# suhrig/arriba

Hardware: AMD Instinct MI355X
Metric: chimeric reads/s end-to-end (BAM->fusions.tsv), synthetic (higher is better)
Workload: dtype int32

## Files before the change

### arriba_amd/csrc/device/agpu_ingest.hip

```cpp
#include <hip/hip_runtime.h>
#include <algorithm>
#include <cstring>
#include <string>
#include <vector>
#include <rocprim/rocprim.hpp>
#include "agpu_context.hpp"
#include "ingest_core.hpp"
#include "device_utils.hpp"
#include "shard_host.hpp"
#include "crc32_core.hpp"
#include "inflate_fast_core.hpp"

using namespace agpu;
namespace agpu { extern thread_local bool g_inside_ingest_finish; }

namespace {

const int BLOCK = 256;
inline unsigned int grid_for(uint64_t n, int block = BLOCK) { return (unsigned int) ((n + block - 1) / block); }

enum { IC_ACTIVE = 0, IC_MAPPED_READS = 1, IC_MISSING_HI = 2, IC_BROKEN = 3, IC_MALFORMED = 4, IC_CHIMERIC = 5, IC_COLLISION = 6, IC_MISMATCH = 7, IC_UNSORTED = 8, IC_MAX_NAME = 9,
       IC_MAX_READ_LENGTH = 10, IC_STRAND_COUNT = 11, IC_STRAND_MATCHING = 12, IC_RUNS_UNSORTED = 13, IC_QNAME_COMMA = 14, IC_COUNT = 16 };

#define HIP_CHECK(call) do { hipError_t e_ = (call); if (e_ != hipSuccess) { set_last_error(std::string(#call) + ": " + hipGetErrorString(e_)); return AGPU_ERR_DEVICE; } } while (0)
// ... 204 lines not shown
__global__ void run_key_kernel(const uint64_t* keys, const uint32_t* group_first, uint32_t n_groups, uint64_t* out) {
	const uint32_t g = blockIdx.x * BLOCK + threadIdx.x;
	if (g < n_groups) out[g] = keys[group_first[g]];
}
__global__ void run_repeat_kernel(const uint64_t* sorted_keys, uint32_t n_groups, uint32_t* repeats) {
	__shared__ uint32_t block_sum;
	uint32_t mine = 0;
	for (uint64_t g = blockIdx.x * (uint64_t) BLOCK + threadIdx.x; g < n_groups; g += gridDim.x * (uint64_t) BLOCK) mine += g > 0 && sorted_keys[g] == sorted_keys[g - 1];
	block_tally(mine, repeats, &block_sum);
}

struct ViralCounter {
	unsigned long long* counts;
	__device__ void operator()(uint32_t contig) { atomicAdd(&counts[contig], 1ull); }
};

#ifndef AGPU_REPLAY_WAVES
#define AGPU_REPLAY_WAVES 0
#endif
#ifndef AGPU_PACK_WAVES
#define AGPU_PACK_WAVES 0
#endif
#if AGPU_REPLAY_WAVES > 0
#define AGPU_REPLAY_OCCUPANCY __attribute__((amdgpu_waves_per_eu(AGPU_REPLAY_WAVES, AGPU_REPLAY_WAVES)))
#else
#define AGPU_REPLAY_OCCUPANCY
#endif
#if AGPU_PACK_WAVES > 0
#define AGPU_PACK_OCCUPANCY __attribute__((amdgpu_waves_per_eu(AGPU_PACK_WAVES, AGPU_PACK_WAVES)))
#else
#define AGPU_PACK_OCCUPANCY
#endif
template <bool RUNS, int ROLE = ROLE_WHOLE> __global__ void __launch_bounds__(BLOCK) AGPU_REPLAY_OCCUPANCY group_replay_kernel(IngestContext ctx, const uint32_t* sorted_records, const uint32_t* group_begin, const uint32_t* group_count, uint32_t first_group, uint32_t n_groups,
                                                             FragmentPlan* plain, TandemPlan* itd, uint8_t* valid, FragmentSizes* sizes, unsigned long long* viral_counts, uint32_t* qname_differs, uint32_t* counters, TakenNames taken) {
	__shared__ uint32_t sums[2];
	GroupTally tally; tally.malformed = 0; tally.chimeric = 0; tally.collision = 0;
	const uint32_t g = first_group + blockIdx.x * BLOCK + threadIdx.x;
	if (g < n_groups) {
		const uint32_t begin = group_begin[g];
		const uint32_t n_records = group_count[g];
		const Rec representative = load_record(ctx.stream, sorted_records[begin]);
		const int64_t hit = hit_index_of(ctx.stream, sorted_records[begin], representative);
		const uint32_t length = qname_length(representative);
		if (RUNS) {
			if (find_byte(representative.name, length, ',') < length) atomicOr(&counters[IC_QNAME_COMMA], 1u);
			if (g == 0) qname_differs[0] = 0;
			else {
				const uint32_t record_before = sorted_records[group_begin[g - 1]];
				const Rec run_before = load_record(ctx.stream, record_before);
				const uint32_t length_before = qname_length(run_before), shorter = length < length_before ? length : length_before, different = first_difference(run_before.name, representative.name, shorter);
				qname_differs[g] = length != length_before || different < shorter;
				bool unsorted;
				if (different < shorter) unsorted = run_before.name[different] > representative.name[different];
				else unsorted = compare_names(fragment_name(run_before, hit_index_of(ctx.stream, record_before, run_before), false, length_before), fragment_name(representative, hit, false, length)) >= 0;
				if (unsorted) atomicOr(&counters[IC_RUNS_UNSORTED], 1u);
			}
		}
		FragmentPlan plain_plan; TandemPlan itd_plan;
		ViralCounter viral = { viral_counts };
		replay_group_as<ROLE>(ctx, sorted_records + begin, n_records, plain_plan, itd_plan, tally, viral, RUNS ? &representative : nullptr, length, hit, taken);
		if (tally.collision) atomicOr(&counters[IC_COLLISION], 1u);
		Fragment3 fragment;
		AGPU_NOUNROLL for (uint32_t entry = 0; entry < 2; ++entry) {
			const FragmentPlan& plan = entry ? itd_plan.plan : plain_plan;
			bool ok = false;
			if (plan.count > 0) {
				ok = normalize_plan(ctx.stream, plan, entry ? &itd_plan.tandem : nullptr, fragment);
				if (!ok) tally.malformed++;
			}
			valid[2 * (size_t) g + entry] = ok;
			FragmentSizes mine; mine.cigar_words = 0; mine.sequence_bytes = 0; mine.name_length = 0;
			if (ok) { if (entry) itd[g] = itd_plan; else plain[g] = plain_plan; fragment_sizes(fragment, representative, hit, entry, mine, length); }
			sizes[2 * (size_t) g + entry] = mine;
		}
	}
	block_tally(tally.malformed, &counters[IC_MALFORMED], &sums[0]);
	block_tally(tally.chimeric, &counters[IC_CHIMERIC], &sums[1]);
}


__device__ FragmentName name_of(const IngestStream& in, const uint32_t* group_first, uint32_t ref, Rec& storage) {
	storage = load_record(in, group_first[ref >> 1]);
	return fragment_name(storage, hit_index_of(in, group_first[ref >> 1], storage), ref & 1);
}

__global__ void name_order_check_kernel(IngestStream in, const uint32_t* group_first, const uint32_t* order, uint64_t n, uint32_t* counters) {
	__shared__ uint32_t block_max;
	if (threadIdx.x == 0) block_max = 0;
	__syncthreads();
	const uint64_t i = blockIdx.x * (uint64_t) BLOCK + threadIdx.x;
	if (i < n) {
		Rec storage_a, storage_b;
		const FragmentName mine = name_of(in, group_first, order[i], storage_a);
		atomicMax(&block_max, name_length(mine));
		if (i > 0) {
			const FragmentName before = name_of(in, group_first, order[i - 1], storage_b);
			if (compare_names(before, mine) >= 0) atomicOr(&counters[IC_UNSORTED], 1u);
		}
	}
	__syncthreads();
	if (threadIdx.x == 0 && block_max) atomicMax(&counters[IC_MAX_NAME], block_max);
}

__global__ void run_itd_order_kernel(IngestStream in, const uint32_t* group_first, const uint8_t* valid, uint32_t first_group, uint32_t n_groups, uint32_t* counters) {
	const uint32_t g = first_group + blockIdx.x * BLOCK + threadIdx.x;
// ... 1 lines not shown
	Rec storage_a, storage_b;
	const FragmentName mine = name_of(in, group_first, 2 * g, storage_b);
	const FragmentName before = name_of(in, group_first, 2 * (g - 1) + 1, storage_a);
	if (compare_names(before, mine) >= 0) atomicOr(&counters[IC_RUNS_UNSORTED], 1u);
}

__global__ void name_chunk_kernel(IngestStream in, const uint32_t* group_first, const uint32_t* order, uint64_t n, uint32_t chunk, uint64_t* keys) {
	const uint64_t i = blockIdx.x * (uint64_t) BLOCK + threadIdx.x;
	if (i >= n) return;
	Rec storage;
	keys[i] = name_chunk(name_of(in, group_first, order[i], storage), chunk);
}


__global__ void fragment_layout_kernel(IngestStream in, const uint32_t* group_first, const uint32_t* order, uint64_t n, const FragmentSizes* sizes, const uint32_t* qname_run ,
                                       uint32_t* cigar_words, uint32_t* sequence_bytes, uint32_t* name_lengths, uint32_t* new_group) {
	const uint64_t i = blockIdx.x * (uint64_t) BLOCK + threadIdx.x;
	if (i > n) return;
	if (i == n) { cigar_words[i] = 0; sequence_bytes[i] = 0; name_lengths[i] = 0; return; }
	const uint32_t ref = order[i];
	const FragmentSizes mine = sizes[ref];
	cigar_words[i] = mine.cigar_words; sequence_bytes[i] = mine.sequence_bytes; name_lengths[i] = mine.name_length;
	uint32_t differs = 0;
	if (i > 0 && qname_run != nullptr) differs = qname_run[ref >> 1] != qname_run[order[i - 1] >> 1];
	else if (i > 0) {
		const Rec a = load_record(in, group_first[ref >> 1]), b = load_record(in, group_first[order[i - 1] >> 1]);
		const uint32_t length = qname_length(a);
		differs = length != qname_length(b);
		for (uint32_t k = 0; k < length && !differs; ++k) differs = a.name[k] != b.name[k];
	}
	new_group[i] = differs;
}

__global__ void __launch_bounds__(BLOCK) AGPU_PACK_OCCUPANCY fragment_pack_kernel(IngestStream in, const uint32_t* group_first, const uint32_t* order, uint64_t n, const FragmentPlan* plain, const TandemPlan* itd,
                                                              const uint64_t* cigar_base, const uint64_t* sequence_base, const uint64_t* name_base, const uint32_t* group_id, PackTarget out, uint32_t* counters) {
	__shared__ uint32_t block_max;
	if (threadIdx.x == 0) block_max = 0;
	__syncthreads();
	const uint64_t i = blockIdx.x * (uint64_t) BLOCK + threadIdx.x;
	if (i == n) out.name_offset[n] = name_base[n];
	if (i < n) {
		const uint32_t ref = order[i], g = ref >> 1;
		const bool is_itd = ref & 1;
		Fragment3 f;
		normalize_plan(in, is_itd ? itd[g].plan : plain[g], is_itd ? &itd[g].tandem : nullptr, f);
		Rec storage;
		const FragmentName name = name_of(in, group_first, ref, storage);
		atomicMax(&block_max, write_fragment(in, f, name, i, cigar_base[i], sequence_base[i], name_base[i], group_id[i], out));
	}
	__syncthreads();
	if (threadIdx.x == 0 && block_max) atomicMax(&counters[IC_MAX_READ_LENGTH], block_max);
}

template <bool INFLATED> __global__ void __launch_bounds__(256) bgzf_crc_kernel(const uint8_t* raw, const agpu_bgzf_block* blocks, uint32_t n_blocks, const Crc32Tables* tables, unsigned int* mismatches) {
	__shared__ uint32_t slice[4][256];
	__shared__ uint32_t join[2][4][256];
	__shared__ uint32_t staged[4][CRC32_WAVE_LANES * (CRC32_ROUND_WORDS + 1)];
	for (uint32_t k = threadIdx.x; k < 4 * 256; k += 256) ((uint32_t*) slice)[k] = ((const uint32_t*) tables->slice)[k];
	for (uint32_t k = threadIdx.x; k < 2 * 4 * 256; k += 256) ((uint32_t*) join)[k] = ((const uint32_t*) tables->join)[k];
	const uint32_t wave = threadIdx.x / CRC32_WAVE_LANES, lane = threadIdx.x % CRC32_WAVE_LANES, b = blockIdx.x * 4 + wave;
	agpu_bgzf_block block;
	block.crc32 = 0; block.payload_size = 0; block.raw_offset = 0; block.payload_offset = 0;
	if (b < n_blocks) block = blocks[b];
	if (INFLATED) { block.raw_offset = block.stream_offset; block.payload_offset = 0; block.payload_size = block.isize; }
	const bool checked = b < n_blocks && block.crc32 != 0 && block.payload_size <= CRC32_VIRTUAL;
	const uint8_t* payload = raw + block.raw_offset + block.payload_offset;
	const uint32_t n = block.payload_size;
	uint32_t* mine = staged[wave];
	uint32_t c = 0;
	const bool by_chunks = checked && n >= 4;
	const uint32_t first_word = by_chunks ? (CRC32_VIRTUAL - n) / 4 : CRC32_VIRTUAL / 4;
	for (uint32_t round = 0; round < CRC32_WAVE_CHUNK / 4 / CRC32_ROUND_WORDS; ++round) {
		__syncthreads();
		for (uint32_t item = lane; item < CRC32_WAVE_LANES * CRC32_ROUND_WORDS; item += CRC32_WAVE_LANES) {
			const uint32_t chunk = item / CRC32_ROUND_WORDS, j = item % CRC32_ROUND_WORDS, w = chunk * (CRC32_WAVE_CHUNK / 4) + round * CRC32_ROUND_WORDS + j;
			mine[chunk * (CRC32_ROUND_WORDS + 1) + j] = w >= first_word ? crc32_virtual_word(payload, n, w) : 0u;
		}
		__syncthreads();
		for (uint32_t j = 0; j < CRC32_ROUND_WORDS; ++j) c = crc32_raw_step(slice, c, mine[lane * (CRC32_ROUND_WORDS + 1) + j]);
	}
	__syncthreads();
// ... 262 lines not shown
		const uint64_t records = w.record_end - w.record_begin;
		w.active_begin = p.active;
		if (records == 0) break;
		DeviceBuffer& record_offset = ctx->scratch("ingest.record_offset"); DeviceBuffer& keys = ctx->scratch("ingest.keys"); DeviceBuffer& record_bits = ctx->scratch("ingest.record_bits"); DeviceBuffer& active_records = ctx->scratch("ingest.sorted_records");
		TRY(grow_keeping(ctx, record_offset, w.record_end * 8, w.record_begin * 8, estimated_records * 8)); TRY(grow_keeping(ctx, keys, w.record_end * 8, w.record_begin * 8, estimated_records * 8));
		TRY(grow_keeping(ctx, ctx->scratch("ingest.hit_index"), w.record_end * 4, w.record_begin * 4, estimated_records * 4));
		TRY(grow_keeping(ctx, record_bits, w.record_end, w.record_begin, estimated_records)); TRY(grow_keeping(ctx, active_records, (w.active_begin + records) * 4, w.active_begin * 4, estimated_records * 4));
		{ KernelTimer timer(ctx, "segment_emit_kernel", records * 8, s);
		  segment_emit_kernel<<<grid_for(n), BLOCK, 0, s>>>(bytes, w.avail, base, w.segment_begin, w.segment_end, ctx->scratch("ingest.segment_first").as<uint64_t>(), ctx->scratch("ingest.segment_base").as<uint32_t>(), record_offset.as<uint64_t>()); }
		const IngestStream in = window_stream(ctx, w.avail, w.record_end);
		{ KernelTimer timer(ctx, "record_parse_kernel", records * (8 + 64 + 9), s);
		  record_parse_kernel<ROLE_WHOLE><<<tally_grid(records, BLOCK) * 8, BLOCK, 0, s>>>(in, ctx->genome, 0, w.record_begin, keys.as<uint64_t>(), record_bits.as<uint8_t>(), ctx->scratch("ingest.hit_index").as<int32_t>(), device_counters); }
		auto flags = rocprim::make_transform_iterator(record_bits.as<uint8_t>() + w.record_begin, RecordIsActive());
		HIP_CHECK(rocprim::select(nullptr, temporary, rocprim::counting_iterator<uint32_t>((uint32_t) w.record_begin), flags, active_records.as<uint32_t>() + w.active_begin, words + 2, records, s));
		if (temporary > rocprim_scratch.capacity) ALLOC(rocprim_scratch, temporary);
		HIP_CHECK(rocprim::select(rocprim_scratch.ptr, temporary, rocprim::counting_iterator<uint32_t>((uint32_t) w.record_begin), flags, active_records.as<uint32_t>() + w.active_begin, words + 2, records, s));
		break; }
	case 3: {
		const uint64_t active = w.active_end - w.active_begin;
		w.head_begin = p.heads;
		if (active == 0) break;
		DeviceBuffer& head = ctx->scratch("ingest.head"); DeviceBuffer& run_begin = ctx->scratch("ingest.group_begin");
		TRY(grow_keeping(ctx, head, w.active_end, 0, estimated_records)); TRY(grow_keeping(ctx, run_begin, (w.head_begin + active + 1) * 4, w.head_begin * 4, estimated_records * 2));
		{ KernelTimer timer(ctx, "run_head_kernel", active * (8 + 4 + 1), s);
		  run_head_kernel<<<grid_for(active), BLOCK, 0, s>>>(ctx->scratch("ingest.keys").as<uint64_t>(), ctx->scratch("ingest.sorted_records").as<uint32_t>(), w.active_begin, w.active_end, head.as<uint8_t>()); }
		HIP_CHECK(rocprim::select(nullptr, temporary, rocprim::counting_iterator<uint32_t>((uint32_t) w.active_begin), head.as<uint8_t>() + w.active_begin, run_begin.as<uint32_t>() + w.head_begin, words + 3, active, s));
		if (temporary > rocprim_scratch.capacity) ALLOC(rocprim_scratch, temporary);
		HIP_CHECK(rocprim::select(rocprim_scratch.ptr, temporary, rocprim::counting_iterator<uint32_t>((uint32_t) w.active_begin), head.as<uint8_t>() + w.active_begin, run_begin.as<uint32_t>() + w.head_begin, words + 3, active, s));
		break; }
	case 4: {
		const uint64_t first_group = p.groups_done, n_groups = w.last ? w.head_end : (w.head_end > 0 ? w.head_end - 1 : 0);
		if (n_groups <= first_group) break;
		DeviceBuffer& group_first = ctx->scratch("ingest.group_first"); DeviceBuffer& group_count = ctx->scratch("ingest.group_count");
		DeviceBuffer& plain = ctx->scratch("ingest.plain_plans"); DeviceBuffer& itd = ctx->scratch("ingest.itd_plans"); DeviceBuffer& valid = ctx->scratch("ingest.valid"); DeviceBuffer& sizes = ctx->scratch("ingest.sizes");
		const size_t estimated_groups = estimated_records / 3;
		TRY(grow_keeping(ctx, group_first, n_groups * 4, first_group * 4, estimated_groups * 4)); TRY(grow_keeping(ctx, group_count, n_groups * 4, first_group * 4, estimated_groups * 4));
		TRY(grow_keeping(ctx, plain, n_groups * sizeof(FragmentPlan), first_group * sizeof(FragmentPlan), estimated_groups * sizeof(FragmentPlan))); TRY(grow_keeping(ctx, itd, n_groups * sizeof(TandemPlan), first_group * sizeof(TandemPlan), estimated_groups * sizeof(TandemPlan)));
		TRY(grow_keeping(ctx, valid, 2 * n_groups, 2 * first_group, 2 * estimated_groups)); TRY(grow_keeping(ctx, sizes, 2 * n_groups * sizeof(FragmentSizes), 2 * first_group * sizeof(FragmentSizes), 2 * estimated_groups * sizeof(FragmentSizes)));
		const uint32_t* active_records = ctx->scratch("ingest.sorted_records").as<uint32_t>(); const uint32_t* run_begin = ctx->scratch("ingest.group_begin").as<uint32_t>();
		const uint64_t groups = n_groups - first_group;
		run_close_kernel<<<grid_for(groups), BLOCK, 0, s>>>(active_records, run_begin, (uint32_t) first_group, (uint32_t) n_groups, (uint32_t) w.head_end, w.active_end, group_first.as<uint32_t>(), group_count.as<uint32_t>());
		const IngestStream in = window_stream(ctx, w.avail, w.record_end);
		DeviceBuffer& qname_differs = ctx->scratch("ingest.qname_differs");
		TRY(grow_keeping(ctx, qname_differs, n_groups * 4, first_group * 4, estimated_groups * 4));
		{ KernelTimer timer(ctx, "group_replay_kernel", n * SEGMENT_BYTES, s);
		  group_replay_kernel<true><<<grid_for(groups), BLOCK, 0, s>>>(replay_context(ctx, in), active_records, run_begin, group_count.as<uint32_t>(), (uint32_t) first_group, (uint32_t) n_groups, plain.as<FragmentPlan>(), itd.as<TandemPlan>(), valid.as<uint8_t>(),
		                                                              sizes.as<FragmentSizes>(), ctx->ingest_viral_counts.as<unsigned long long>(), qname_differs.as<uint32_t>(), device_counters, TakenNames()); }
		{ KernelTimer timer(ctx, "run_itd_order_kernel", groups * 2, s);
		  run_itd_order_kernel<<<grid_for(groups), BLOCK, 0, s>>>(in, group_first.as<uint32_t>(), valid.as<uint8_t>(), (uint32_t) first_group, (uint32_t) n_groups, device_counters); }
		p.groups_done = n_groups; p.touched = true;
		break; }
	}
	HIP_CHECK(hipMemcpyAsync(p.host_words + (size_t) w.slot * INGEST_WINDOW_WORDS, words, INGEST_WINDOW_WORDS * 4, hipMemcpyDeviceToHost, s));
	HIP_CHECK(hipEventRecord(w.readback, s));
	++w.enqueued;
	return AGPU_OK;
}

void window_note(agpu_ctx* ctx, IngestWindow& w) {
	IngestProgress& p = ctx->ingest_progress;
	const uint32_t* words = p.host_words + (size_t) w.slot * INGEST_WINDOW_WORDS;
	w.known = w.enqueued;
	switch (w.known) {
	case 1: {
		w.record_begin = p.records;
		if (w.segment_end == w.segment_begin) { w.record_end = p.records; break; }
		const uint64_t last_end = (uint64_t) words[4] | (uint64_t) words[5] << 32;
		if (words[0] != 0 || last_end >= OFFSET_BROKEN || (w.last && last_end != w.avail)) { p.abandoned = true; break; }
		w.record_end = words[1]; p.records = w.record_end;
		break; }
	case 2: w.active_end = w.active_begin + (w.record_end > w.record_begin ? words[2] : 0); p.active = w.active_end; break;
	case 3: w.head_end = w.head_begin + (w.active_end > w.active_begin ? words[3] : 0); p.heads = w.head_end; break;
	}
}

int windows_advance(agpu_ctx* ctx, bool wait) {
	IngestProgress& p = ctx->ingest_progress;
	while (!p.abandoned && !p.windows.empty()) {
		bool moved = false;
// ... 487 lines not shown
			TRY(sort_pairs<uint64_t>(ctx, rocprim_scratch, keys.as<uint64_t>(), keys_sorted.as<uint64_t>(), nullptr, sorted_records.as<uint32_t>(), n_records, 64, "rocprim::radix_sort_pairs(record keys)", true));
		}
		TRY(read_counters());
		if (host_counters[IC_BROKEN] > 0) { set_last_error(ctx->ingest_role == AGPU_ROLE_SEPARATE_CHIMERIC ? "failed to load alignments: a record of the separate chimeric file (-c) is damaged or has no reference sequence" : "failed to load alignments"); return AGPU_ERR_INVALID; }
		n_active = host_counters[IC_ACTIVE];
		n_groups = 0;
		if (n_active > 0) {
			ALLOC(head, n_active); ALLOC(group_start, (n_active + 1) * 4);
			{ KernelTimer timer(ctx, "group_head_kernel", n_active * (8 + 1));
			  group_head_kernel<<<grid_for(n_active), BLOCK, 0, s>>>(keys_sorted.as<uint64_t>(), n_active, head.as<uint8_t>()); }
			TRY(select_flagged(ctx, rocprim_scratch, head.as<uint8_t>(), group_start.as<uint32_t>(), device_counters + IC_MAX_NAME , n_active));
			TRY(read_counters());
			n_groups = host_counters[IC_MAX_NAME];
			HIP_CHECK(hipMemsetAsync(device_counters + IC_MAX_NAME, 0, 4, s));
			ALLOC(first_flags, n_records); ALLOC(stream_rank, (n_records + 1) * 4); ALLOC(group_first, (size_t) n_groups * 4); ALLOC(group_begin, (size_t) n_groups * 4); ALLOC(group_count, (size_t) n_groups * 4);
			HIP_CHECK(hipMemsetAsync(first_flags.ptr, 0, n_records, s));
			group_first_flag_kernel<<<grid_for(n_groups), BLOCK, 0, s>>>(sorted_records.as<uint32_t>(), group_start.as<uint32_t>(), n_groups, first_flags.as<uint8_t>());
			{ size_t scan_bytes = 0;
			  HIP_CHECK(rocprim::exclusive_scan(nullptr, scan_bytes, first_flags.as<uint8_t>(), stream_rank.as<uint32_t>(), 0u, n_records, rocprim::plus<uint32_t>(), s));
			  if (scan_bytes > rocprim_scratch.capacity) ALLOC(rocprim_scratch, scan_bytes);
			  KernelTimer timer(ctx, "rocprim::exclusive_scan(first records)", n_records * 5);
			  HIP_CHECK(rocprim::exclusive_scan(rocprim_scratch.ptr, scan_bytes, first_flags.as<uint8_t>(), stream_rank.as<uint32_t>(), 0u, n_records, rocprim::plus<uint32_t>(), s)); }
			{ KernelTimer timer(ctx, "group_rank_kernel", (uint64_t) n_groups * 24);
			  group_rank_kernel<<<grid_for(n_groups), BLOCK, 0, s>>>(sorted_records.as<uint32_t>(), group_start.as<uint32_t>(), n_groups, n_active, stream_rank.as<uint32_t>(), group_first.as<uint32_t>(), group_begin.as<uint32_t>(), group_count.as<uint32_t>()); }
			{ KernelTimer timer(ctx, "group_names_kernel", n_active * (4 + 36 + 16));
			  group_names_kernel<<<grid_for(n_groups), BLOCK, 0, s>>>(in, sorted_records.as<uint32_t>(), group_begin.as<uint32_t>(), group_count.as<uint32_t>(), 0, n_groups, device_counters); }
			TRY(read_counters());
			if (host_counters[IC_COLLISION]) { seed += 0x632BE59BD9B4E019ull; continue; }
		}
		break;
	}
	const uint64_t mapped_reads = host_counters[IC_MAPPED_READS], missing_hi_tag = host_counters[IC_MISSING_HI];

	DeviceBuffer& plain = ctx->scratch("ingest.plain_plans"); DeviceBuffer& itd = ctx->scratch("ingest.itd_plans"); DeviceBuffer& valid = ctx->scratch("ingest.valid"); DeviceBuffer& sizes = ctx->scratch("ingest.sizes");
	DeviceBuffer& refs = ctx->scratch("ingest.refs"); DeviceBuffer& order = ctx->scratch("ingest.order"); DeviceBuffer& order_keys = ctx->scratch("ingest.order_keys"); DeviceBuffer& order_keys_sorted = ctx->scratch("ingest.order_keys_sorted");
	const uint64_t groups1 = std::max<uint32_t>(n_groups, 1);
	ALLOC(plain, groups1 * sizeof(FragmentPlan)); ALLOC(itd, groups1 * sizeof(TandemPlan)); ALLOC(valid, 2 * groups1); ALLOC(sizes, 2 * groups1 * sizeof(FragmentSizes));
	ALLOC(refs, 2 * groups1 * 4);
	uint64_t n_fragments = 0;
	if (n_groups > 0) {
		if (!streamed && ctx->ingest_role == AGPU_ROLE_SEPARATE_CHIMERIC) { KernelTimer timer(ctx, "group_replay_kernel(separate chimeric)", size - base);
		  group_replay_kernel<false, ROLE_SEPARATE_CHIMERIC><<<grid_for(n_groups), BLOCK, 0, s>>>(replay_context(ctx, in), sorted_records.as<uint32_t>(), group_begin.as<uint32_t>(), group_count.as<uint32_t>(), 0, n_groups, plain.as<FragmentPlan>(), itd.as<TandemPlan>(), valid.as<uint8_t>(),
		                                                            sizes.as<FragmentSizes>(), ctx->ingest_viral_counts.as<unsigned long long>(), nullptr, device_counters, TakenNames()); }
		else if (!streamed && ctx->ingest_role == AGPU_ROLE_SEPARATE_RNA) { KernelTimer timer(ctx, "group_replay_kernel(separate rna)", size - base);
		  TakenNames taken;
		  taken.keys = ctx->separate_keys.as<uint64_t>(); taken.rows = ctx->separate_rows.as<uint32_t>(); taken.n = ctx->separate_n;
		  taken.names = ctx->separate_block.as<char>() + ctx->separate_names_at; taken.name_offset = (const uint64_t*) (ctx->separate_block.as<uint8_t>() + ctx->separate_name_offset_at);
		  group_replay_kernel<false, ROLE_SEPARATE_RNA><<<grid_for(n_groups), BLOCK, 0, s>>>(replay_context(ctx, in), sorted_records.as<uint32_t>(), group_begin.as<uint32_t>(), group_count.as<uint32_t>(), 0, n_groups, plain.as<FragmentPlan>(), itd.as<TandemPlan>(), valid.as<uint8_t>(),
		                                                            sizes.as<FragmentSizes>(), ctx->ingest_viral_counts.as<unsigned long long>(), nullptr, device_counters, taken); }
		else if (!streamed) { KernelTimer timer(ctx, "group_replay_kernel", size - base);
		  group_replay_kernel<false><<<grid_for(n_groups), BLOCK, 0, s>>>(replay_context(ctx, in), sorted_records.as<uint32_t>(), group_begin.as<uint32_t>(), group_count.as<uint32_t>(), 0, n_groups, plain.as<FragmentPlan>(), itd.as<TandemPlan>(), valid.as<uint8_t>(),
		                                                            sizes.as<FragmentSizes>(), ctx->ingest_viral_counts.as<unsigned long long>(), nullptr, device_counters, TakenNames()); }
		TRY(select_flagged(ctx, rocprim_scratch, valid.as<uint8_t>(), refs.as<uint32_t>(), device_counters + IC_MAX_NAME, 2 * (uint64_t) n_groups));
		TRY(read_counters());
		n_fragments = host_counters[IC_MAX_NAME];
		HIP_CHECK(hipMemsetAsync(device_counters + IC_MAX_NAME, 0, 4, s));
	} else TRY(read_counters());
	const uint64_t malformed_count = host_counters[IC_MALFORMED];
	const bool no_chimeric_reads = host_counters[IC_CHIMERIC] == 0;
	if (n_fragments >= 0xFFFFFFF0ull) { set_last_error("a batch holds at most 2^32-16 fragments; shard larger inputs"); return AGPU_ERR_INVALID; }
	const uint64_t fragments1 = std::max<uint64_t>(n_fragments, 1);
	bool names_were_sorted = true;
	ALLOC(order, fragments1 * 4);
	if (n_fragments > 0) {
		ALLOC(order_keys, fragments1 * 8); ALLOC(order_keys_sorted, fragments1 * 8);
		HIP_CHECK(hipMemcpyAsync(order.ptr, refs.ptr, n_fragments * 4, hipMemcpyDeviceToDevice, s));
		const bool runs_in_name_order = streamed && host_counters[IC_RUNS_UNSORTED] == 0;
		if (!runs_in_name_order) {
			KernelTimer timer(ctx, "name_order_check_kernel", n_fragments * (4 + 2 * 40));
			name_order_check_kernel<<<grid_for(n_fragments), BLOCK, 0, s>>>(in, group_first.as<uint32_t>(), order.as<uint32_t>(), n_fragments, device_counters);
		}
		TRY(read_counters());
		if (!runs_in_name_order && host_counters[IC_UNSORTED]) {
			names_were_sorted = false;
			const uint32_t chunks = (host_counters[IC_MAX_NAME] + 7) / 8;
			for (uint32_t chunk = chunks; chunk-- > 0; ) {
				{ KernelTimer timer(ctx, "name_chunk_kernel", n_fragments * (4 + 8 + 40));
				  name_chunk_kernel<<<grid_for(n_fragments), BLOCK, 0, s>>>(in, group_first.as<uint32_t>(), order.as<uint32_t>(), n_fragments, chunk, order_keys.as<uint64_t>()); }
				TRY(sort_pairs<uint64_t>(ctx, rocprim_scratch, order_keys.as<uint64_t>(), order_keys_sorted.as<uint64_t>(), order.as<uint32_t>(), refs.as<uint32_t>(), n_fragments, 64, "rocprim::radix_sort_pairs(name chunk)", false));
				order.swap(refs);
			}
		}
	}

// ... 8 lines not shown
		size_t scan_bytes = 0;
		HIP_CHECK(rocprim::inclusive_scan(nullptr, scan_bytes, qname_differs.as<uint32_t>(), numbered.as<uint32_t>(), n_groups, rocprim::plus<uint32_t>(), s));
		if (scan_bytes > rocprim_scratch.capacity) ALLOC(rocprim_scratch, scan_bytes);
		HIP_CHECK(rocprim::inclusive_scan(rocprim_scratch.ptr, scan_bytes, qname_differs.as<uint32_t>(), numbered.as<uint32_t>(), n_groups, rocprim::plus<uint32_t>(), s));
		qname_run = numbered.as<uint32_t>();
	}
	{ KernelTimer timer(ctx, "fragment_layout_kernel", n_fragments * (4 + 8 + 16 + (qname_run ? 8 : 2 * 40)));
	  fragment_layout_kernel<<<grid_for(n_fragments + 1), BLOCK, 0, s>>>(in, group_first.as<uint32_t>(), order.as<uint32_t>(), n_fragments, sizes.as<FragmentSizes>(), qname_run,
	                                                                   cigar_words.as<uint32_t>(), sequence_bytes.as<uint32_t>(), name_lengths.as<uint32_t>(), new_group.as<uint32_t>()); }
	TRY(exclusive_sum_u64(ctx, rocprim_scratch, cigar_words.as<uint32_t>(), cigar_base.as<uint64_t>(), n_fragments + 1));
	TRY(exclusive_sum_u64(ctx, rocprim_scratch, sequence_bytes.as<uint32_t>(), sequence_base.as<uint64_t>(), n_fragments + 1));
	TRY(exclusive_sum_u64(ctx, rocprim_scratch, name_lengths.as<uint32_t>(), name_base.as<uint64_t>(), n_fragments + 1));
	if (n_fragments > 0) {
		size_t scan_bytes = 0;
		HIP_CHECK(rocprim::inclusive_scan(nullptr, scan_bytes, new_group.as<uint32_t>(), group_id.as<uint32_t>(), n_fragments, rocprim::plus<uint32_t>(), s));
		if (scan_bytes > rocprim_scratch.capacity) ALLOC(rocprim_scratch, scan_bytes);
		HIP_CHECK(rocprim::inclusive_scan(rocprim_scratch.ptr, scan_bytes, new_group.as<uint32_t>(), group_id.as<uint32_t>(), n_fragments, rocprim::plus<uint32_t>(), s));
	}
	uint64_t totals[3] = { 0, 0, 0 };
	HIP_CHECK(hipMemcpyAsync(&totals[0], cigar_base.as<uint64_t>() + n_fragments, 8, hipMemcpyDeviceToHost, s));
	HIP_CHECK(hipMemcpyAsync(&totals[1], sequence_base.as<uint64_t>() + n_fragments, 8, hipMemcpyDeviceToHost, s));
	HIP_CHECK(hipMemcpyAsync(&totals[2], name_base.as<uint64_t>() + n_fragments, 8, hipMemcpyDeviceToHost, s));
	HIP_CHECK(hipStreamSynchronize(s));
	if (totals[0] >= 0xFFFFFFFFull || totals[1] / 4 >= 0xFFFFFFFFull) { set_last_error("batch too large for 32-bit pool offsets"); return AGPU_ERR_INVALID; }
	const uint64_t n = n_fragments;
	ctx->n = n;
	ALLOC(ctx->n_aln, n); ALLOC(ctx->fbits, n); ALLOC(ctx->group, n * 4);
	for (int k = 0; k < 3; ++k) { ALLOC(ctx->contig[k], n * 2); ALLOC(ctx->start[k], n * 4); ALLOC(ctx->end[k], n * 4); ALLOC(ctx->abits[k], n); ALLOC(ctx->cigar_offset[k], n * 4); ALLOC(ctx->cigar_count[k], n * 2); }
	for (int k = 0; k < 2; ++k) { ALLOC(ctx->seq_offset[k], n * 4); ALLOC(ctx->seq_length[k], n * 4); }
	ALLOC(ctx->cigar_pool, totals[0] * 4); ALLOC(ctx->seq_pool, totals[1]); ALLOC(ctx->names, totals[2]); ALLOC(ctx->name_offset, (n + 1) * 8);
	ctx->names_size = totals[2]; ctx->ingest_pool_sizes[0] = totals[0]; ctx->ingest_pool_sizes[1] = totals[1];
	PackTarget target;
	fill_pack_target(ctx, target);
	{ KernelTimer timer(ctx, "fragment_pack_kernel", n * (1 + 1 + 4 + 3 * 17 + 16 + 4 + 24) + totals[0] * 8 + totals[1] * 2 + totals[2] * 2);
	  fragment_pack_kernel<<<grid_for(n + 1), BLOCK, 0, s>>>(in, group_first.as<uint32_t>(), order.as<uint32_t>(), n, plain.as<FragmentPlan>(), itd.as<TandemPlan>(),
	                                                       cigar_base.as<uint64_t>(), sequence_base.as<uint64_t>(), name_base.as<uint64_t>(), group_id.as<uint32_t>(), target, device_counters); }
	const uint64_t windows = ctx->host_coverage_window_offset.empty() ? 0 : ctx->host_coverage_window_offset.back();
	if (windows > 0) {
		const uint64_t slots = coverage_difference_slots(windows, ctx->genome.n_contigs);
		DeviceBuffer& summed = ctx->scratch("ingest.coverage_summed"); DeviceBuffer& rocprim_scratch = ctx->scratch("ingest.rocprim");
		ALLOC(summed, slots * 4);
		size_t temporary = 0;
		HIP_CHECK(rocprim::inclusive_scan(nullptr, temporary, ctx->coverage_windows32.as<uint32_t>(), summed.as<uint32_t>(), slots, rocprim::plus<uint32_t>(), s));
		ALLOC(rocprim_scratch, temporary);
		KernelTimer timer(ctx, "coverage_from_differences_kernel", slots * 8 + windows * 10);
		HIP_CHECK(rocprim::inclusive_scan(rocprim_scratch.ptr, temporary, ctx->coverage_windows32.as<uint32_t>(), summed.as<uint32_t>(), slots, rocprim::plus<uint32_t>(), s));
		coverage_from_differences_kernel<<<grid_for(windows), BLOCK, 0, s>>>(summed.as<uint32_t>(), ctx->coverage_window_offset.as<uint64_t>(), ctx->genome.n_contigs, windows, ctx->coverage_windows32.as<uint32_t>(), ctx->coverage_windows.as<uint16_t>());
	}
	TRY(read_counters());
	HIP_CHECK(hipEventRecord(ctx->event_stop, s));
	HIP_CHECK(hipEventSynchronize(ctx->event_stop));
	HIP_CHECK(hipEventElapsedTime(&ctx->last_ms, ctx->event_start, ctx->event_stop));
	collect_kernel_samples(ctx);
	ctx->last_bytes = (size - base) * 2 + n_records * 40 + n * 250;
	ctx->max_read_length = host_counters[IC_MAX_READ_LENGTH];
	ctx->batch_input_bytes = n * (1 + 1 + 4 + 3 * 17 + 16) + totals[0] * 4 + totals[1];
	ctx->coverage.n_contigs = ctx->genome.n_contigs; ctx->coverage.window_offset = ctx->coverage_window_offset.as<uint64_t>(); ctx->coverage.coverage = ctx->coverage_windows.as<uint16_t>();
	ctx->coverage.fragment_starts = ctx->coverage_fragment_starts.as<uint8_t>(); ctx->coverage.fragment_ends = ctx->coverage_fragment_ends.as<uint8_t>();
	ctx->have_coverage = true;
	TRY(agpu::finish_batch_setup(ctx));
	ctx->batch_from_ingest = true;
	if (getenv("ARRIBA_RELEASE_INGEST_BUFFERS") != nullptr) agpu::release_ingest_buffers(ctx);
	ctx->last_ingest_stream_size = size; ctx->last_ingest_first_record = base; ctx->last_ingest_records = n_records; ctx->last_ingest_part_of_sample = ctx->ingest_part_of_sample;
	ctx->last_ingest_kept = ctx->ingest_stream.ptr != nullptr && record_offset.ptr != nullptr;
	ctx->ingest_stream_size = 0;
	agpu_ingest_result& mine = ctx->ingest_result;
	memset(&mine, 0, sizeof(mine));
	mine.records = n_records; mine.fragments = n; mine.mapped_reads = mapped_reads; mine.malformed_count = malformed_count; mine.missing_hi_tag = missing_hi_tag;
// ... 559 lines not shown
```

### arriba_amd/csrc/device/ingest_core.hpp

```cpp
#ifndef AGPU_INGEST_CORE_HPP
#define AGPU_INGEST_CORE_HPP 1

#include "annotate_core.hpp"
#include "event_core.hpp"

namespace agpu {


AGPU_HD uint32_t load_u32(const uint8_t* p) { uint32_t v; __builtin_memcpy(&v, p, 4); return v; }
AGPU_HD uint64_t load_u64(const uint8_t* p) { uint64_t v; __builtin_memcpy(&v, p, 8); return v; }
AGPU_HD uint32_t first_zero_byte(uint64_t v) { const uint64_t z = (v - 0x0101010101010101ull) & ~v & 0x8080808080808080ull; return z ? (uint32_t) __builtin_ctzll(z) >> 3 : 8u; }
AGPU_HD uint64_t low_bytes(uint32_t n) { return n >= 8 ? ~0ull : (1ull << (8 * n)) - 1; }
AGPU_HD uint32_t find_byte(const uint8_t* p, uint32_t n, uint8_t byte) {
	const uint64_t pattern = 0x0101010101010101ull * byte;
	uint32_t i = 0;
	for (; i + 8 <= n; i += 8) { const uint32_t z = first_zero_byte(load_u64(p + i) ^ pattern); if (z < 8) return i + z; }
	if (i == n) return n;
	if (n >= 8) {
		const uint32_t z = first_zero_byte((load_u64(p + n - 8) ^ pattern) | low_bytes(i - (n - 8)));
		return z < 8 ? n - 8 + z : n;
	}
	for (; i < n; ++i) if (p[i] == byte) return i;
	return n;
}
// ... 920 lines not shown
		cigar_at += a.n_cigar;
		if (s < 2) {
			const uint32_t length = (uint32_t) a.sequence_length, bytes = (length + 1) / 2, padded = padded_sequence_bytes(length);
			out.seq_offset[s][i] = (uint32_t) (sequence_at / 4); out.seq_length[s][i] = length;
			if (length > longest) longest = length;
			if (length > 0) {
				const Rec source = load_record(in, a.sequence_record);
				uint32_t* target = (uint32_t*) (out.seq_pool + sequence_at);
				for (uint32_t w = 0; w < padded / 4; ++w) {
					uint32_t value = 0;
					if (4 * w + 4 < bytes) value = load_u32(source.seq_bytes + 4 * w);
					else for (uint32_t b = 0; b < 4; ++b) {
						const uint32_t at = 4 * w + b;
						if (at >= bytes) break;
						uint32_t byte = source.seq_bytes[at];
						if (at == bytes - 1 && (length & 1)) byte &= 0xF0u;
						value |= byte << (8 * b);
					}
					target[w] = value;
				}
			}
			sequence_at += padded;
		}
	}
	out.name_offset[i] = name_at;
	const uint32_t length = name_length(name);
	uint32_t copied = 0;
	for (; copied + 8 <= name.qname_length; copied += 8) { const uint64_t word = load_u64(name.qname + copied); __builtin_memcpy(out.names + name_at + copied, &word, 8); }
	for (uint32_t k = copied; k < name.qname_length; ++k) out.names[name_at + k] = (char) name.qname[k];
	for (uint32_t k = name.qname_length; k < length; ++k) out.names[name_at + k] = (char) name_byte(name, k);
	return longest;
}

AGPU_HD void row_sizes(const BatchView& b, const uint64_t* name_offset, uint64_t i, uint32_t& cigar_words, uint32_t& sequence_bytes, uint32_t& name_bytes) {
	cigar_words = 0; sequence_bytes = 0;
	for (uint32_t s = 0; s < b.n_aln[i]; ++s) {
		cigar_words += b.cigar_count[s][i];
		if (s < 2) sequence_bytes += padded_sequence_bytes(b.seq_length[s][i]);
	}
	name_bytes = name_offset ? (uint32_t) (name_offset[i + 1] - name_offset[i]) : 0;
}
AGPU_HD void copy_row(const BatchView& b, const uint8_t* pristine_fbits, const uint8_t* const* pristine_abits, const uint64_t* name_offset, const char* names, uint64_t i, uint64_t k,
                      uint64_t cigar_at, uint64_t sequence_at, uint64_t name_at, const PackTarget& out) {
	const uint32_t n_aln = b.n_aln[i];
	out.n_aln[k] = (uint8_t) n_aln; out.fbits[k] = pristine_fbits[i]; out.group[k] = b.group[i];
	for (uint32_t s = 0; s < 3; ++s) {
		out.contig[s][k] = b.contig[s][i]; out.start[s][k] = b.start[s][i]; out.end[s][k] = b.end[s][i]; out.abits[s][k] = pristine_abits[s][i];
		const uint32_t count = s < n_aln ? b.cigar_count[s][i] : 0;
		out.cigar_count[s][k] = (uint16_t) count; out.cigar_offset[s][k] = s < n_aln ? (uint32_t) cigar_at : 0;
		for (uint32_t c = 0; c < count; ++c) out.cigar_pool[cigar_at + c] = b.cigar_pool[b.cigar_offset[s][i] + c];
		cigar_at += count;
		if (s < 2) {
			const uint32_t length = s < n_aln ? b.seq_length[s][i] : 0, padded = padded_sequence_bytes(length);
			out.seq_length[s][k] = length; out.seq_offset[s][k] = s < n_aln ? (uint32_t) (sequence_at / 4) : 0;
			if (length > 0) {
				const uint32_t* source = (const uint32_t*) b.seq_pool + b.seq_offset[s][i];
				uint32_t* target = (uint32_t*) (out.seq_pool + sequence_at);
				for (uint32_t w = 0; w < padded / 4; ++w) target[w] = source[w];
			}
			sequence_at += padded;
		}
	}
	if (out.name_offset) out.name_offset[k] = name_at; else out.row_name_offset[k] = (uint32_t) name_at;
	if (name_offset) for (uint64_t c = name_offset[i]; c < name_offset[i + 1]; ++c) out.names[name_at + (c - name_offset[i])] = names[c];
}

// ... 20 lines not shown
```

Measured before the change: 60.81 million.

## Replace stored fragment plans with compact summaries and wave-cooperative pool packing

The replay kernel now writes a fixed 160-byte FragmentSummary per fragment slot (offsets into the stream, edge cigar words, coordinates, name metadata) instead of full FragmentPlan/TandemPlan structs. The pack kernel stops re-running normalize_plan and record loads per fragment. Each wave stages 64 summaries and their base offsets in shared memory, then writes the cigar, sequence and name pools cooperatively as coalesced 32-bit words, finding each word's owner by binary search. The aim is to cut redundant re-normalization and uncoalesced per-thread byte copies, at the cost of extra shared memory, binary searches per output word, and a larger summary buffer indexed as 2 per group.

```diff
diff --git a/arriba_amd/csrc/device/agpu_ingest.hip b/arriba_amd/csrc/device/agpu_ingest.hip
--- a/arriba_amd/csrc/device/agpu_ingest.hip
+++ b/arriba_amd/csrc/device/agpu_ingest.hip
@@ -260,7 +260,7 @@
 #define AGPU_PACK_OCCUPANCY
 #endif
 template <bool RUNS, int ROLE = ROLE_WHOLE> __global__ void __launch_bounds__(BLOCK) AGPU_REPLAY_OCCUPANCY group_replay_kernel(IngestContext ctx, const uint32_t* sorted_records, const uint32_t* group_begin, const uint32_t* group_count, uint32_t first_group, uint32_t n_groups,
-                                                             FragmentPlan* plain, TandemPlan* itd, uint8_t* valid, FragmentSizes* sizes, unsigned long long* viral_counts, uint32_t* qname_differs, uint32_t* counters, TakenNames taken) {
+                                                             FragmentSummary* summaries, uint8_t* valid, FragmentSizes* sizes, unsigned long long* viral_counts, uint32_t* qname_differs, uint32_t* counters, TakenNames taken) {
 	__shared__ uint32_t sums[2];
 	GroupTally tally; tally.malformed = 0; tally.chimeric = 0; tally.collision = 0;
 	const uint32_t g = first_group + blockIdx.x * BLOCK + threadIdx.x;
@@ -298,7 +298,7 @@
 			}
 			valid[2 * (size_t) g + entry] = ok;
 			FragmentSizes mine; mine.cigar_words = 0; mine.sequence_bytes = 0; mine.name_length = 0;
-			if (ok) { if (entry) itd[g] = itd_plan; else plain[g] = plain_plan; fragment_sizes(fragment, representative, hit, entry, mine, length); }
+			if (ok) { fragment_sizes(fragment, representative, hit, entry, mine, length); summarize(ctx.stream, fragment, representative, hit, entry, length, summaries[2 * (size_t) g + entry]); }
 			sizes[2 * (size_t) g + entry] = mine;
 		}
 	}
@@ -366,21 +366,43 @@
 	new_group[i] = differs;
 }
 
-__global__ void __launch_bounds__(BLOCK) AGPU_PACK_OCCUPANCY fragment_pack_kernel(IngestStream in, const uint32_t* group_first, const uint32_t* order, uint64_t n, const FragmentPlan* plain, const TandemPlan* itd,
+const uint32_t PACK_WAVE = 64, PACK_WAVES = BLOCK / PACK_WAVE;
+__global__ void __launch_bounds__(BLOCK) AGPU_PACK_OCCUPANCY fragment_pack_kernel(IngestStream in, const uint32_t* order, uint64_t n, const FragmentSummary* summaries,
                                                               const uint64_t* cigar_base, const uint64_t* sequence_base, const uint64_t* name_base, const uint32_t* group_id, PackTarget out, uint32_t* counters) {
+	__shared__ FragmentSummary summary[BLOCK];
+	__shared__ uint64_t base[PACK_WAVES][3][PACK_WAVE + 1];
 	__shared__ uint32_t block_max;
 	if (threadIdx.x == 0) block_max = 0;
+	const uint32_t wave = threadIdx.x / PACK_WAVE, lane = threadIdx.x % PACK_WAVE;
+	const uint64_t i = blockIdx.x * (uint64_t) BLOCK + threadIdx.x, first = i - lane;
+	const uint32_t count = first < n ? (uint32_t) (n - first < PACK_WAVE ? n - first : PACK_WAVE) : 0;
 	__syncthreads();
-	const uint64_t i = blockIdx.x * (uint64_t) BLOCK + threadIdx.x;
 	if (i == n) out.name_offset[n] = name_base[n];
-	if (i < n) {
-		const uint32_t ref = order[i], g = ref >> 1;
-		const bool is_itd = ref & 1;
-		Fragment3 f;
-		normalize_plan(in, is_itd ? itd[g].plan : plain[g], is_itd ? &itd[g].tandem : nullptr, f);
-		Rec storage;
-		const FragmentName name = name_of(in, group_first, ref, storage);
-		atomicMax(&block_max, write_fragment(in, f, name, i, cigar_base[i], sequence_base[i], name_base[i], group_id[i], out));
+	if (lane < count) {
+		const uint64_t cigar_at = cigar_base[i], sequence_at = sequence_base[i], name_at = name_base[i];
+		base[wave][0][lane] = cigar_at; base[wave][1][lane] = sequence_at; base[wave][2][lane] = name_at;
+		if (lane == 0) { base[wave][0][count] = cigar_base[first + count]; base[wave][1][count] = sequence_base[first + count]; base[wave][2][count] = name_base[first + count]; }
+		FragmentSummary& mine = summary[threadIdx.x];
+		mine = summaries[order[i]];
+		atomicMax(&block_max, write_summary_columns(mine, i, cigar_at, sequence_at, name_at, group_id[i], out));
+	}
+	__syncthreads();
+	if (count > 0) {
+		SummaryTile tile;
+		tile.stream = in.bytes; tile.fragment = summary + wave * PACK_WAVE; tile.cigar_base = base[wave][0]; tile.sequence_base = base[wave][1]; tile.name_base = base[wave][2]; tile.count = count;
+		for (uint64_t w = tile.cigar_base[0] + lane; w < tile.cigar_base[count]; w += PACK_WAVE) out.cigar_pool[w] = tile_cigar_word(tile, w);
+		uint32_t* sequence_words = (uint32_t*) out.seq_pool;
+		for (uint64_t w = tile.sequence_base[0] / 4 + lane; w < tile.sequence_base[count] / 4; w += PACK_WAVE) sequence_words[w] = tile_sequence_word(tile, w);
+		const uint64_t begin = tile.name_base[0], end = tile.name_base[count], skew = (uint64_t) (uintptr_t) out.names & 3;
+		if (end > begin) {
+			for (uint64_t q = (begin + skew) / 4 + lane; q <= (end + skew - 1) / 4; q += PACK_WAVE) {
+				uint64_t word_begin, word_end;
+				tile_name_span(begin, end, skew, q, word_begin, word_end);
+				const uint32_t bytes = (uint32_t) (word_end - word_begin), value = tile_name_bytes(tile, word_begin, bytes);
+				if (bytes == 4) *(uint32_t*) (out.names + word_begin) = value;
+				else for (uint32_t b = 0; b < bytes; ++b) out.names[word_begin + b] = (char) (value >> (8 * b));
+			}
+		}
 	}
 	__syncthreads();
 	if (threadIdx.x == 0 && block_max) atomicMax(&counters[IC_MAX_READ_LENGTH], block_max);
@@ -709,10 +731,10 @@
 		const uint64_t first_group = p.groups_done, n_groups = w.last ? w.head_end : (w.head_end > 0 ? w.head_end - 1 : 0);
 		if (n_groups <= first_group) break;
 		DeviceBuffer& group_first = ctx->scratch("ingest.group_first"); DeviceBuffer& group_count = ctx->scratch("ingest.group_count");
-		DeviceBuffer& plain = ctx->scratch("ingest.plain_plans"); DeviceBuffer& itd = ctx->scratch("ingest.itd_plans"); DeviceBuffer& valid = ctx->scratch("ingest.valid"); DeviceBuffer& sizes = ctx->scratch("ingest.sizes");
+		DeviceBuffer& summaries = ctx->scratch("ingest.summaries"); DeviceBuffer& valid = ctx->scratch("ingest.valid"); DeviceBuffer& sizes = ctx->scratch("ingest.sizes");
 		const size_t estimated_groups = estimated_records / 3;
 		TRY(grow_keeping(ctx, group_first, n_groups * 4, first_group * 4, estimated_groups * 4)); TRY(grow_keeping(ctx, group_count, n_groups * 4, first_group * 4, estimated_groups * 4));
-		TRY(grow_keeping(ctx, plain, n_groups * sizeof(FragmentPlan), first_group * sizeof(FragmentPlan), estimated_groups * sizeof(FragmentPlan))); TRY(grow_keeping(ctx, itd, n_groups * sizeof(TandemPlan), first_group * sizeof(TandemPlan), estimated_groups * sizeof(TandemPlan)));
+		TRY(grow_keeping(ctx, summaries, 2 * n_groups * sizeof(FragmentSummary), 2 * first_group * sizeof(FragmentSummary), 2 * estimated_groups * sizeof(FragmentSummary)));
 		TRY(grow_keeping(ctx, valid, 2 * n_groups, 2 * first_group, 2 * estimated_groups)); TRY(grow_keeping(ctx, sizes, 2 * n_groups * sizeof(FragmentSizes), 2 * first_group * sizeof(FragmentSizes), 2 * estimated_groups * sizeof(FragmentSizes)));
 		const uint32_t* active_records = ctx->scratch("ingest.sorted_records").as<uint32_t>(); const uint32_t* run_begin = ctx->scratch("ingest.group_begin").as<uint32_t>();
 		const uint64_t groups = n_groups - first_group;
@@ -721,7 +743,7 @@
 		DeviceBuffer& qname_differs = ctx->scratch("ingest.qname_differs");
 		TRY(grow_keeping(ctx, qname_differs, n_groups * 4, first_group * 4, estimated_groups * 4));
 		{ KernelTimer timer(ctx, "group_replay_kernel", n * SEGMENT_BYTES, s);
-		  group_replay_kernel<true><<<grid_for(groups), BLOCK, 0, s>>>(replay_context(ctx, in), active_records, run_begin, group_count.as<uint32_t>(), (uint32_t) first_group, (uint32_t) n_groups, plain.as<FragmentPlan>(), itd.as<TandemPlan>(), valid.as<uint8_t>(),
+		  group_replay_kernel<true><<<grid_for(groups), BLOCK, 0, s>>>(replay_context(ctx, in), active_records, run_begin, group_count.as<uint32_t>(), (uint32_t) first_group, (uint32_t) n_groups, summaries.as<FragmentSummary>(), valid.as<uint8_t>(),
 		                                                              sizes.as<FragmentSizes>(), ctx->ingest_viral_counts.as<unsigned long long>(), qname_differs.as<uint32_t>(), device_counters, TakenNames()); }
 		{ KernelTimer timer(ctx, "run_itd_order_kernel", groups * 2, s);
 		  run_itd_order_kernel<<<grid_for(groups), BLOCK, 0, s>>>(in, group_first.as<uint32_t>(), valid.as<uint8_t>(), (uint32_t) first_group, (uint32_t) n_groups, device_counters); }
@@ -1275,24 +1297,24 @@
 	}
 	const uint64_t mapped_reads = host_counters[IC_MAPPED_READS], missing_hi_tag = host_counters[IC_MISSING_HI];
 
-	DeviceBuffer& plain = ctx->scratch("ingest.plain_plans"); DeviceBuffer& itd = ctx->scratch("ingest.itd_plans"); DeviceBuffer& valid = ctx->scratch("ingest.valid"); DeviceBuffer& sizes = ctx->scratch("ingest.sizes");
+	DeviceBuffer& summaries = ctx->scratch("ingest.summaries"); DeviceBuffer& valid = ctx->scratch("ingest.valid"); DeviceBuffer& sizes = ctx->scratch("ingest.sizes");
 	DeviceBuffer& refs = ctx->scratch("ingest.refs"); DeviceBuffer& order = ctx->scratch("ingest.order"); DeviceBuffer& order_keys = ctx->scratch("ingest.order_keys"); DeviceBuffer& order_keys_sorted = ctx->scratch("ingest.order_keys_sorted");
 	const uint64_t groups1 = std::max<uint32_t>(n_groups, 1);
-	ALLOC(plain, groups1 * sizeof(FragmentPlan)); ALLOC(itd, groups1 * sizeof(TandemPlan)); ALLOC(valid, 2 * groups1); ALLOC(sizes, 2 * groups1 * sizeof(FragmentSizes));
+	ALLOC(summaries, 2 * groups1 * sizeof(FragmentSummary)); ALLOC(valid, 2 * groups1); ALLOC(sizes, 2 * groups1 * sizeof(FragmentSizes));
 	ALLOC(refs, 2 * groups1 * 4);
 	uint64_t n_fragments = 0;
 	if (n_groups > 0) {
 		if (!streamed && ctx->ingest_role == AGPU_ROLE_SEPARATE_CHIMERIC) { KernelTimer timer(ctx, "group_replay_kernel(separate chimeric)", size - base);
-		  group_replay_kernel<false, ROLE_SEPARATE_CHIMERIC><<<grid_for(n_groups), BLOCK, 0, s>>>(replay_context(ctx, in), sorted_records.as<uint32_t>(), group_begin.as<uint32_t>(), group_count.as<uint32_t>(), 0, n_groups, plain.as<FragmentPlan>(), itd.as<TandemPlan>(), valid.as<uint8_t>(),
+		  group_replay_kernel<false, ROLE_SEPARATE_CHIMERIC><<<grid_for(n_groups), BLOCK, 0, s>>>(replay_context(ctx, in), sorted_records.as<uint32_t>(), group_begin.as<uint32_t>(), group_count.as<uint32_t>(), 0, n_groups, summaries.as<FragmentSummary>(), valid.as<uint8_t>(),
 		                                                            sizes.as<FragmentSizes>(), ctx->ingest_viral_counts.as<unsigned long long>(), nullptr, device_counters, TakenNames()); }
 		else if (!streamed && ctx->ingest_role == AGPU_ROLE_SEPARATE_RNA) { KernelTimer timer(ctx, "group_replay_kernel(separate rna)", size - base);
 		  TakenNames taken;
 		  taken.keys = ctx->separate_keys.as<uint64_t>(); taken.rows = ctx->separate_rows.as<uint32_t>(); taken.n = ctx->separate_n;
 		  taken.names = ctx->separate_block.as<char>() + ctx->separate_names_at; taken.name_offset = (const uint64_t*) (ctx->separate_block.as<uint8_t>() + ctx->separate_name_offset_at);
-		  group_replay_kernel<false, ROLE_SEPARATE_RNA><<<grid_for(n_groups), BLOCK, 0, s>>>(replay_context(ctx, in), sorted_records.as<uint32_t>(), group_begin.as<uint32_t>(), group_count.as<uint32_t>(), 0, n_groups, plain.as<FragmentPlan>(), itd.as<TandemPlan>(), valid.as<uint8_t>(),
+		  group_replay_kernel<false, ROLE_SEPARATE_RNA><<<grid_for(n_groups), BLOCK, 0, s>>>(replay_context(ctx, in), sorted_records.as<uint32_t>(), group_begin.as<uint32_t>(), group_count.as<uint32_t>(), 0, n_groups, summaries.as<FragmentSummary>(), valid.as<uint8_t>(),
 		                                                            sizes.as<FragmentSizes>(), ctx->ingest_viral_counts.as<unsigned long long>(), nullptr, device_counters, taken); }
 		else if (!streamed) { KernelTimer timer(ctx, "group_replay_kernel", size - base);
-		  group_replay_kernel<false><<<grid_for(n_groups), BLOCK, 0, s>>>(replay_context(ctx, in), sorted_records.as<uint32_t>(), group_begin.as<uint32_t>(), group_count.as<uint32_t>(), 0, n_groups, plain.as<FragmentPlan>(), itd.as<TandemPlan>(), valid.as<uint8_t>(),
+		  group_replay_kernel<false><<<grid_for(n_groups), BLOCK, 0, s>>>(replay_context(ctx, in), sorted_records.as<uint32_t>(), group_begin.as<uint32_t>(), group_count.as<uint32_t>(), 0, n_groups, summaries.as<FragmentSummary>(), valid.as<uint8_t>(),
 		                                                            sizes.as<FragmentSizes>(), ctx->ingest_viral_counts.as<unsigned long long>(), nullptr, device_counters, TakenNames()); }
 		TRY(select_flagged(ctx, rocprim_scratch, valid.as<uint8_t>(), refs.as<uint32_t>(), device_counters + IC_MAX_NAME, 2 * (uint64_t) n_groups));
 		TRY(read_counters());
@@ -1367,8 +1389,8 @@
 	ctx->names_size = totals[2]; ctx->ingest_pool_sizes[0] = totals[0]; ctx->ingest_pool_sizes[1] = totals[1];
 	PackTarget target;
 	fill_pack_target(ctx, target);
-	{ KernelTimer timer(ctx, "fragment_pack_kernel", n * (1 + 1 + 4 + 3 * 17 + 16 + 4 + 24) + totals[0] * 8 + totals[1] * 2 + totals[2] * 2);
-	  fragment_pack_kernel<<<grid_for(n + 1), BLOCK, 0, s>>>(in, group_first.as<uint32_t>(), order.as<uint32_t>(), n, plain.as<FragmentPlan>(), itd.as<TandemPlan>(),
+	{ KernelTimer timer(ctx, "fragment_pack_kernel", n * (1 + 1 + 4 + 3 * 17 + 16 + 4 + 24 + sizeof(FragmentSummary)) + totals[0] * 8 + totals[1] * 2 + totals[2] * 2);
+	  fragment_pack_kernel<<<grid_for(n + 1), BLOCK, 0, s>>>(in, order.as<uint32_t>(), n, summaries.as<FragmentSummary>(),
 	                                                       cigar_base.as<uint64_t>(), sequence_base.as<uint64_t>(), name_base.as<uint64_t>(), group_id.as<uint32_t>(), target, device_counters); }
 	const uint64_t windows = ctx->host_coverage_window_offset.empty() ? 0 : ctx->host_coverage_window_offset.back();
 	if (windows > 0) {
diff --git a/arriba_amd/csrc/device/ingest_core.hpp b/arriba_amd/csrc/device/ingest_core.hpp
--- a/arriba_amd/csrc/device/ingest_core.hpp
+++ b/arriba_amd/csrc/device/ingest_core.hpp
@@ -976,6 +976,145 @@
 	return longest;
 }
 
+struct alignas(16) FragmentSummary {
+	uint64_t cigar_at[3];
+	uint64_t sequence_at[2];
+	uint64_t name_at;
+	uint32_t edge[3][4];
+	int32_t start[3], end[3];
+	uint32_t n_cigar[3];
+	uint32_t sequence_length[2];
+	uint32_t hit_magnitude;
+	uint16_t contig[3];
+	uint8_t abits[3];
+	uint8_t bits;
+	uint8_t qname_length;
+	uint8_t reserved[5];
+};
+static_assert(sizeof(FragmentSummary) == 160, "FragmentSummary: ten 16-byte words");
+enum : uint8_t { SUMMARY_N_MASK = 3, SUMMARY_SINGLE_END = 4, SUMMARY_DUPLICATE = 8, SUMMARY_ITD = 16, SUMMARY_HIT_NEGATIVE = 32 };
+
+AGPU_HD void summarize(const IngestStream& in, const Fragment3& f, const Rec& representative, int64_t hit_index , bool itd, uint32_t length , FragmentSummary& out) {
+	for (uint32_t s = 0; s < 3; ++s) {
+		out.cigar_at[s] = 0; out.start[s] = 0; out.end[s] = 0; out.n_cigar[s] = 0; out.contig[s] = 0; out.abits[s] = 0;
+		for (uint32_t k = 0; k < 4; ++k) out.edge[s][k] = 0;
+		if (s < 2) { out.sequence_at[s] = 0; out.sequence_length[s] = 0; }
+		if (s >= f.n) continue;
+		const Aln& a = f.a[s];
+		const uint32_t n = a.n_cigar;
+		out.cigar_at[s] = (uint64_t) ((int64_t) (a.cigar_bytes - in.bytes) + 4 * (int64_t) (int32_t) a.shift);
+		out.start[s] = a.start; out.end[s] = a.end; out.n_cigar[s] = n; out.contig[s] = (uint16_t) a.contig;
+		out.abits[s] = (a.strand ? ABIT_STRAND : 0) | (a.first_in_pair ? ABIT_FIRST_IN_PAIR : 0) | (a.supplementary ? ABIT_SUPPLEMENTARY : 0) | ABIT_PREDICTED_STRAND_AMBIGUOUS;
+		out.edge[s][0] = a.cigar(0); out.edge[s][3] = a.cigar(n - 1);
+		if (n > 1) { out.edge[s][1] = a.cigar(1); out.edge[s][2] = a.cigar(n - 2); }
+		if (s < 2) {
+			out.sequence_length[s] = (uint32_t) a.sequence_length;
+			if (a.sequence_length > 0) out.sequence_at[s] = (uint64_t) (load_record(in, a.sequence_record).seq_bytes - in.bytes);
+		}
+	}
+	out.name_at = (uint64_t) (representative.name - in.bytes);
+	out.hit_magnitude = (uint32_t) (hit_index < 0 ? (uint64_t) (-(hit_index + 1)) + 1 : (uint64_t) hit_index);
+	out.bits = (uint8_t) ((f.n & SUMMARY_N_MASK) | (f.single_end ? SUMMARY_SINGLE_END : 0) | (f.duplicate ? SUMMARY_DUPLICATE : 0) | (itd ? SUMMARY_ITD : 0) | (hit_index < 0 ? SUMMARY_HIT_NEGATIVE : 0));
+	out.qname_length = (uint8_t) length;
+	for (uint32_t k = 0; k < 5; ++k) out.reserved[k] = 0;
+}
+
+AGPU_HD uint32_t summary_cigar(const uint8_t* stream, const FragmentSummary& f, uint32_t s, uint32_t k) {
+	const uint32_t n = f.n_cigar[s];
+	if (k < 2) return f.edge[s][k];
+	if (n - k <= 2) return f.edge[s][4 - (n - k)];
+	return load_u32(stream + f.cigar_at[s] + 4 * (uint64_t) k);
+}
+AGPU_HD uint32_t decimal_length(uint32_t magnitude) { uint32_t n = 1; while (magnitude >= 10) { magnitude /= 10; ++n; } return n; }
+AGPU_HD uint32_t summary_name_length(const FragmentSummary& f) {
+	return (uint32_t) f.qname_length + 1 + ((f.bits & SUMMARY_HIT_NEGATIVE) ? 1 : 0) + decimal_length(f.hit_magnitude) + ((f.bits & SUMMARY_ITD) ? 3 : 0);
+}
+AGPU_HD uint8_t summary_name_byte(const uint8_t* stream, const FragmentSummary& f, uint32_t k ) {
+	if (k < f.qname_length) return stream[f.name_at + k];
+	k -= f.qname_length;
+	if (k == 0) return ',';
+	--k;
+	if (f.bits & SUMMARY_HIT_NEGATIVE) { if (k == 0) return '-'; --k; }
+	const uint32_t digits = decimal_length(f.hit_magnitude);
+	if (k < digits) { uint32_t m = f.hit_magnitude; for (uint32_t d = digits - 1 - k; d > 0; --d) m /= 10; return (uint8_t) ('0' + m % 10); }
+	k -= digits;
+	return k == 0 ? 'I' : k == 1 ? 'T' : 'D';
+}
+AGPU_HD void summary_sizes(const FragmentSummary& f, FragmentSizes& sizes) {
+	sizes.cigar_words = f.n_cigar[0] + f.n_cigar[1] + f.n_cigar[2];
+	sizes.sequence_bytes = padded_sequence_bytes(f.sequence_length[0]) + padded_sequence_bytes(f.sequence_length[1]);
+	sizes.name_length = summary_name_length(f);
+}
+AGPU_HD uint32_t write_summary_columns(const FragmentSummary& f, uint64_t i, uint64_t cigar_at, uint64_t sequence_at, uint64_t name_at, uint32_t group, const PackTarget& out) {
+	const uint32_t n = f.bits & SUMMARY_N_MASK;
+	out.n_aln[i] = (uint8_t) n;
+	out.fbits[i] = ((f.bits & SUMMARY_SINGLE_END) ? FBIT_SINGLE_END : 0) | ((f.bits & SUMMARY_DUPLICATE) ? FBIT_DUPLICATE : 0);
+	out.group[i] = group;
+	const uint32_t first = f.n_cigar[0], second = f.n_cigar[1];
+	out.contig[0][i] = f.contig[0]; out.start[0][i] = f.start[0]; out.end[0][i] = f.end[0]; out.abits[0][i] = f.abits[0]; out.cigar_offset[0][i] = (uint32_t) cigar_at; out.cigar_count[0][i] = (uint16_t) first;
+	out.contig[1][i] = f.contig[1]; out.start[1][i] = f.start[1]; out.end[1][i] = f.end[1]; out.abits[1][i] = f.abits[1]; out.cigar_offset[1][i] = (uint32_t) (cigar_at + first); out.cigar_count[1][i] = (uint16_t) second;
+	out.contig[2][i] = f.contig[2]; out.start[2][i] = f.start[2]; out.end[2][i] = f.end[2]; out.abits[2][i] = f.abits[2]; out.cigar_offset[2][i] = n > 2 ? (uint32_t) (cigar_at + first + second) : 0u; out.cigar_count[2][i] = (uint16_t) f.n_cigar[2];
+	out.seq_offset[0][i] = (uint32_t) (sequence_at / 4); out.seq_length[0][i] = f.sequence_length[0];
+	out.seq_offset[1][i] = (uint32_t) ((sequence_at + padded_sequence_bytes(f.sequence_length[0])) / 4); out.seq_length[1][i] = f.sequence_length[1];
+	out.name_offset[i] = name_at;
+	return f.sequence_length[0] > f.sequence_length[1] ? f.sequence_length[0] : f.sequence_length[1];
+}
+
+struct SummaryTile {
+	const uint8_t* stream;
+	const FragmentSummary* fragment;
+	const uint64_t* cigar_base;
+	const uint64_t* sequence_base;
+	const uint64_t* name_base;
+	uint32_t count;
+};
+AGPU_HD uint32_t tile_owner(const uint64_t* base, uint32_t count, uint64_t at) {
+	uint32_t low = 0, high = count;
+	while (high - low > 1) { const uint32_t middle = (low + high) / 2; if (base[middle] <= at) low = middle; else high = middle; }
+	return low;
+}
+AGPU_HD uint32_t tile_cigar_word(const SummaryTile& t, uint64_t w ) {
+	const uint32_t j = tile_owner(t.cigar_base, t.count, w);
+	const FragmentSummary& f = t.fragment[j];
+	uint32_t k = (uint32_t) (w - t.cigar_base[j]), s = 0;
+	if (k >= f.n_cigar[0]) { k -= f.n_cigar[0]; s = 1; if (k >= f.n_cigar[1]) { k -= f.n_cigar[1]; s = 2; } }
+	return summary_cigar(t.stream, f, s, k);
+}
+AGPU_HD uint32_t tile_sequence_word(const SummaryTile& t, uint64_t w ) {
+	const uint32_t j = tile_owner(t.sequence_base, t.count, 4 * w);
+	const FragmentSummary& f = t.fragment[j];
+	uint32_t offset = (uint32_t) (4 * w - t.sequence_base[j]), s = 0;
+	const uint32_t first = padded_sequence_bytes(f.sequence_length[0]);
+	if (offset >= first) { offset -= first; s = 1; }
+	const uint32_t length = f.sequence_length[s], bytes = (length + 1) / 2;
+	const uint8_t* source = t.stream + f.sequence_at[s];
+	if (offset + 4 < bytes) return load_u32(source + offset);
+	uint32_t value = 0;
+	for (uint32_t b = 0; b < 4; ++b) {
+		const uint32_t at = offset + b;
+		if (at >= bytes) break;
+		uint32_t byte = source[at];
+		if (at == bytes - 1 && (length & 1)) byte &= 0xF0u;
+		value |= byte << (8 * b);
+	}
+	return value;
+}
+AGPU_HD void tile_name_span(uint64_t begin, uint64_t end, uint64_t skew, uint64_t q, uint64_t& from, uint64_t& to) {
+	from = 4 * q > begin + skew ? 4 * q - skew : begin;
+	to = 4 * q + 4 < end + skew ? 4 * q + 4 - skew : end;
+}
+AGPU_HD uint32_t tile_name_bytes(const SummaryTile& t, uint64_t at, uint32_t n) {
+	uint32_t j = tile_owner(t.name_base, t.count, at);
+	uint32_t k = (uint32_t) (at - t.name_base[j]);
+	if (n == 4 && k + 4 <= t.fragment[j].qname_length) return load_u32(t.stream + t.fragment[j].name_at + k);
+	uint32_t value = 0;
+	for (uint32_t b = 0; b < n; ++b) {
+		while (at + b >= t.name_base[j + 1]) { ++j; k = 0; }
+		value |= (uint32_t) summary_name_byte(t.stream, t.fragment[j], k++) << (8 * b);
+	}
+	return value;
+}
+
 AGPU_HD void row_sizes(const BatchView& b, const uint64_t* name_offset, uint64_t i, uint32_t& cigar_words, uint32_t& sequence_bytes, uint32_t& name_bytes) {
 	cigar_words = 0; sequence_bytes = 0;
 	for (uint32_t s = 0; s < b.n_aln[i]; ++s) {
```

After: 58.05 million. 4.5% lower.
